# mic-rud/RABBIT-Transcoding

Hardware: AMD Instinct MI355X
Metric: transcoded point-cloud frames/sec, R5->R3 (higher is better)
Workload: dtype u16/i32

## Files before the change

rabbit-transcoding_amd/csrc/rbt_encode.h:

```cpp
#pragma once
#include "rbt_cabac.h"
#include "rbt_recon.h"
#include "rbt_filter.h"
#include "rbt_qpmap.h"

RBT_CONST uint16_t k_lambda16[76] = {3,    3,    4,    4,    5,    5,    6,    7,    8,    9,    10,   11,   12,   14,   15,   17,   19,   22,   24,
                                     27,   30,   34,   38,   43,   48,   54,   61,   68,   77,   86,   97,   108,  122,  137,  153,  172,  193,  217,
                                     244,  273,  307,  344,  387,  434,  487,  547,  614,  689,  773,  868,  974,  1093, 1227, 1378, 1546, 1736, 1948,
                                     2187, 2454, 2755, 3092, 3471, 3896, 4373, 4909, 5510, 6185, 6942, 7792, 8747, 9818, 11020, 12370, 13884, 15585, 17493};
RBT_CONST uint8_t k_intra_cand[11] = {0, 1, 26, 10, 2, 6, 14, 18, 22, 30, 34};
#define RBT_SPLIT_BITS 48
#define RBT_PARTIAL_COST 0x0FFFFFFF
#define RBT_AN_GOOD 2
#define RBT_AN_SKIPPED 0x0FFFFFFE

struct RbtEncLds {
  RbtReconLds rc;
  int16_t lvl[32 * 32];
};
struct RbtEntropyLds {
  uint8_t scan[3][4][64];
  uint8_t cu_l2[81], cu_md[81], cu_fl[81];
  alignas(16) int16_t lv[64 * 64 * 3 / 2];
};
// ... 1135 lines not shown
    while (st < 4 && (x + (st & 1) * h >= s->w || y + (st >> 1) * h >= s->h)) st++;
    if (st < 4) {
      states = (states & ~(15u << (4 * lvl))) | ((uint32_t)(st + 1) << (4 * lvl));
      x += (st & 1) * h; y += (st >> 1) * h; lg--; lvl++;
      states = (states & ~(15u << (4 * lvl))) | (15u << (4 * lvl));
    } else {
      if (lvl == 0) break;
      lvl--;
      const int k = (int)((states >> (4 * lvl)) & 15u) - 1, hh = 1 << lg;
      x -= (k & 1) * hh; y -= (k >> 1) * hh; lg++;
    }
  }
}
struct RbtSaoLds { int32_t bcnt[8][32], bsum[8][32]; int32_t ecnt[16], esum[16]; int32_t off[3][48], gain[48]; long long tgain[3][5]; int32_t bpos[3]; };
template <int TL2> struct RbtSaoRegionT { uint16_t ry[((1 << TL2) + 8) * ((1 << TL2) + 8)]; uint16_t rc[2][((1 << TL2) / 2 + 4) * ((1 << TL2) / 2 + 4)]; };
RBT_DEV int en_sao_round_div(int sum, int cnt) { return cnt ? (sum >= 0 ? sum + cnt / 2 : sum - cnt / 2) / cnt : 0; }
RBT_DEV void en_wave_sum16(const int (&v)[16], RBT_LDS_AS int32_t* dst) {
#ifdef RBT_HOSTEMU
  for (int q = 0; q < 16; q++) dst[q] = v[q];
#else
  const int lane = (int)threadIdx.x & 63, b0 = lane & 1, b1 = lane & 2;
  int a[8], b[4];
#pragma unroll
  for (int k = 0; k < 8; k++) { const int keep = b0 ? v[k + 8] : v[k], send = b0 ? v[k] : v[k + 8]; a[k] = keep + __builtin_amdgcn_update_dpp(0, send, 0xB1, 0xF, 0xF, false); }
#pragma unroll
  for (int k = 0; k < 4; k++) { const int keep = b1 ? a[k + 4] : a[k], send = b1 ? a[k] : a[k + 4]; b[k] = keep + __builtin_amdgcn_update_dpp(0, send, 0x4E, 0xF, 0xF, false); }
#pragma unroll
  for (int k = 0; k < 4; k++) {
    b[k] += __builtin_amdgcn_update_dpp(0, b[k], 0x124, 0xF, 0xF, false);
    b[k] += __builtin_amdgcn_update_dpp(0, b[k], 0x128, 0xF, 0xF, false);
    b[k] += __builtin_amdgcn_ds_swizzle(b[k], 0x401F);
    b[k] += __builtin_amdgcn_ds_bpermute((lane ^ 32) << 2, b[k]);
  }
  if (lane < 4) {
#pragma unroll
    for (int k = 0; k < 4; k++) dst[(lane & 1) * 8 + (lane & 2) * 2 + k] = b[k];
  }
#endif
}
template <bool REGION, bool QPMAP = EN_QP_ASK> RBT_DEV void en_sao_ctb(RbtFrame* f, const RbtSlice* slices, int ctb_addr, RBT_LDS_AS RbtSaoLds* L, RBT_LDS_AS uint16_t* ry, RBT_LDS_AS uint16_t* rc0, RBT_LDS_AS uint16_t* rc1) {
  const RbtStreamCfg gcopy = rc_cfg_uni(&f->cfg); const RbtStreamCfg* g = &gcopy;
  const int ctb = 1 << g->log2_ctb, cxi = ctb_addr % g->w_ctb, cyi = ctb_addr / g->w_ctb, bd = g->bit_depth, has_occ = RBT_UNI(f->occ4 != nullptr);
  const int flat = RBT_UNI(f->chroma_flat) != 0;
  EN_FLAT_COUNT(2, flat);
  const RbtSlice* sl = &slices[f->ctb_slice[ctb_addr]];
  const long long lam16 = k_lambda16[rbt_clip3(0, 75, en_ctb_qp<QPMAP>(f, sl, ctb_addr) + 6 * (bd - 8))], lam = lam16 * lam16;
  int all_skip = 0;
  if (f->ref_frame >= 0) {
    const int n8 = ctb >> 3; uint64_t m0 = 0, m1 = 0;
    RBT_VBALLOT(m0, p, rbt_min(64, n8 * n8), (cxi * n8 + p % n8 >= f->w8) || (cyi * n8 + p / n8 >= f->h8) || (f->cu_flags[(cyi * n8 + p / n8) * f->w8 + cxi * n8 + p % n8] & RBT_CU_SKIP));
    m1 = n8 * n8 >= 64 ? ~0ull : (1ull << (n8 * n8)) - 1;
    all_skip = m0 == m1;
  }
  const int lx0 = cxi * ctb, ly0 = cyi * ctb, ox = lx0 - 4, oy = ly0 - 4, cox = lx0 / 2 - 2, coy = ly0 / 2 - 2, RS = ctb + 8, RSC = ctb / 2 + 4;
  if constexpr (REGION) {
    RBT_PAR_FOR(i, RS * RS) { const int x = ox + i % RS, y = oy + i / RS; ry[i] = (x >= 0 && y >= 0 && x < g->w && y < g->h) ? f->pix[0][(size_t)y * g->w + x] : 0; }
    RBT_PAR_FOR(i, 2 * RSC * RSC) {
      const int c = i / (RSC * RSC), j = i % (RSC * RSC), x = cox + j % RSC, y = coy + j / RSC;
      (c ? rc1 : rc0)[j] = (x >= 0 && y >= 0 && x < g->cw && y < g->ch) ? f->pix[1 + c][(size_t)y * g->cw + x] : 0;
    }
    RBT_SYNC_LDS();
    for (int dir = 0; dir < 2 && REGION; dir++) {
      const int ne = ctb / 8 + 1, ns = RS / 4;
      RBT_PAR_FOR(i, ne * ns) {
        const int e = i / ns, sg = i % ns;
        const int x = dir == 0 ? lx0 + 8 * e : ox + 4 * sg, y = dir == 0 ? oy + 4 * sg : ly0 + 8 * e;
        if (x >= 0 && y >= 0 && x < g->w && y < g->h) {
          const int bs = fl_bs(f, slices, x, y, dir);
          if (bs) {
            fl_luma_core(f, slices, x, y, dir, bs, &ry[(y - oy) * RS + (x - ox)], dir == 0 ? 1 : RS, dir == 0 ? RS : 1);
            if (bs == 2 && !(dir == 0 ? (x & 15) : (y & 15)))
              for (int c = 0; c < 2; c++) fl_chroma_core(f, slices, 1 + c, x, y, dir, &(c ? rc1 : rc0)[((y >> 1) - coy) * RSC + ((x >> 1) - cox)], dir == 0 ? 1 : RSC, dir == 0 ? RSC : 1);
          }
        }
      }
      RBT_SYNC_LDS();
    }
  }
#define EN_SAO_RP(c, x, y) (REGION ? ((c) == 0 ? (int)ry[((y) - oy) * RS + ((x) - ox)] : (int)((c) == 1 ? rc0 : rc1)[((y) - coy) * RSC + ((x) - cox)]) : (int)f->pix[c][(size_t)(y) * pw + (x)])
  for (int c = 0; c < (flat ? 1 : 3) && !all_skip; c++) {
    const int sh = c ? 1 : 0, pw = c ? g->cw : g->w, ph = c ? g->ch : g->h, n = ctb >> sh, lgn = g->log2_ctb - sh;
    const int x0 = (cxi * ctb) >> sh, y0 = (cyi * ctb) >> sh;
    const uint16_t* sp = f->src[c];
    RBT_PAR_FOR(i, 8 * 32) { L->bcnt[i >> 5][i & 31] = 0; L->bsum[i >> 5][i & 31] = 0; }
    RBT_SYNC_LDS();
    int ecnt[16], esum[16];
#pragma unroll
    for (int q = 0; q < 16; q++) { ecnt[q] = 0; esum[q] = 0; }
    const int interior = !REGION && x0 > 0 && y0 > 0 && x0 + n < pw && y0 + n < ph;
    if (interior) {
#ifdef RBT_HOSTEMU
      typedef long long EnSaoAcc; const int ash = 13;
#else
      typedef int EnSaoAcc; const int ash = 7;
#endif
      EnSaoAcc acc[16];
#pragma unroll
      for (int q = 0; q < 16; q++) acc[q] = 0;
      const uint16_t* rp = f->pix[c];
      RBT_PAR_FOR(i, n * n) {
        const int x = x0 + (i & (n - 1)), y = y0 + (i >> lgn);
        if (!has_occ || en_occ_unit(f, (x << sh) >> 2, (y << sh) >> 2)) {
          const size_t o = (size_t)y * pw + x;
          const int v = rp[o], d = (int)sp[o] - v, b = rbt_min(31, v >> (bd - 5)), copy = i & 7; const EnSaoAcc dp = (EnSaoAcc)d * (1 << ash) + 1;
          RBT_LDS_ADD(&L->bcnt[copy][b], 1); RBT_LDS_ADD(&L->bsum[copy][b], d);
#pragma unroll
          for (int cls = 0; cls < 4; cls++) {
            const int step = cls == 0 ? -1 : (cls == 1 ? -pw : (cls == 2 ? -pw - 1 : -pw + 1));
            const int va = rp[o + step], vb = rp[o - step];
            const int k = 2 + (v > va) - (v < va) + (v > vb) - (v < vb), cat = k < 2 ? k : k - 1;
#pragma unroll
            for (int q = 0; q < 4; q++) acc[cls * 4 + q] += (k != 2 && cat == q) ? dp : (EnSaoAcc)0;
          }
        }
      }
#pragma unroll
      for (int q = 0; q < 16; q++) { ecnt[q] = (int)(acc[q] & ((1 << ash) - 1)); esum[q] = (int)(acc[q] >> ash); }
    } else
    RBT_PAR_FOR(i, n * n) {
      const int x = x0 + (i & (n - 1)), y = y0 + (i >> lgn);
      if (x < pw && y < ph && (!has_occ || en_occ_unit(f, (x << sh) >> 2, (y << sh) >> 2))) {
        const int v = EN_SAO_RP(c, x, y), d = (int)sp[(size_t)y * pw + x] - v, b = rbt_min(31, v >> (bd - 5)), copy = i & 7;
        RBT_LDS_ADD(&L->bcnt[copy][b], 1); RBT_LDS_ADD(&L->bsum[copy][b], d);
#pragma unroll
        for (int cls = 0; cls < 4; cls++) {
          const int dxa = cls == 1 ? 0 : (cls == 3 ? 1 : -1), dya = cls == 0 ? 0 : -1, xa = x + dxa, ya = y + dya, xb = x - dxa, yb = y - dya;
          const int inside = !(xa < 0 || ya < 0 || xb < 0 || yb < 0 || xa >= pw || xb >= pw || ya >= ph || yb >= ph);
          const int va = EN_SAO_RP(c, rbt_clip3(0, pw - 1, xa), rbt_clip3(0, ph - 1, ya)), vb = EN_SAO_RP(c, rbt_clip3(0, pw - 1, xb), rbt_clip3(0, ph - 1, yb));
          const int k = 2 + (v > va) - (v < va) + (v > vb) - (v < vb), cat = k < 2 ? k : k - 1;
#pragma unroll
          for (int q = 0; q < 4; q++) { const int hit = inside && k != 2 && cat == q; ecnt[cls * 4 + q] += hit; esum[cls * 4 + q] += hit ? d : 0; }
        }
      }
    }
    en_wave_sum16(ecnt, L->ecnt); en_wave_sum16(esum, L->esum);
    RBT_SYNC_LDS();
    RBT_PAR_FOR(j, 48) {
      int cnt, sum, o;
      if (j < 32) { cnt = 0; sum = 0; for (int q = 0; q < 8; q++) { cnt += L->bcnt[q][j]; sum += L->bsum[q][j]; } o = rbt_clip3(-7, 7, en_sao_round_div(sum, cnt)); }
      else { cnt = L->ecnt[j - 32]; sum = L->esum[j - 32]; o = en_sao_round_div(sum, cnt); o = ((j - 32) & 3) < 2 ? rbt_clip3(0, 7, o) : rbt_clip3(-7, 0, o); }
      L->off[c][j] = o; L->gain[j] = 2 * o * sum - cnt * o * o;
    }
    RBT_SYNC_LDS();
    { long long best = -1; int bp = 0;
      for (int b = 0; b <= 28; b++) { const long long gsum = (long long)L->gain[b] + L->gain[b + 1] + L->gain[b + 2] + L->gain[b + 3]; if (gsum > best) { best = gsum; bp = b; } }
      if (RBT_LANE0) { L->bpos[c] = bp; L->tgain[c][0] = best * 256 - lam * 18; } }
    for (int cls = 0; cls < 4; cls++) {
      long long gs = 0;
      for (int k = 0; k < 4; k++) gs += L->gain[32 + cls * 4 + k];
      if (RBT_LANE0) L->tgain[c][1 + cls] = gs * 256 - lam * 12;
    }
    RBT_SYNC_LDS();
  }
  RbtSao out; for (int i = 0; i < (int)sizeof(out); i++) ((uint8_t*)&out)[i] = 0;
  int bt = -1; long long bgn = 0;
  if (!all_skip) for (int t = 0; t < 5; t++) if (L->tgain[0][t] > bgn) { bgn = L->tgain[0][t]; bt = t; }
  if (bt >= 0) { out.type[0] = bt == 0 ? 1 : 2; out.band_pos[0] = (uint8_t)(bt == 0 ? L->bpos[0] : 0); out.eo_class[0] = (uint8_t)(bt ? bt - 1 : 0);
    for (int k = 0; k < 4; k++) out.offset[0][k] = (int8_t)(bt == 0 ? L->off[0][L->bpos[0] + k] : L->off[0][32 + (bt - 1) * 4 + k]); }
  bt = -1; bgn = 0;
  if (!all_skip && !flat) for (int t = 0; t < 5; t++) if (L->tgain[1][t] + L->tgain[2][t] > bgn) { bgn = L->tgain[1][t] + L->tgain[2][t]; bt = t; }
  if (bt >= 0) for (int c = 1; c < 3; c++) { out.type[c] = bt == 0 ? 1 : 2; out.band_pos[c] = (uint8_t)(bt == 0 ? L->bpos[c] : 0); out.eo_class[c] = (uint8_t)(bt ? bt - 1 : 0);
    for (int k = 0; k < 4; k++) out.offset[c][k] = (int8_t)(bt == 0 ? L->off[c][L->bpos[c] + k] : L->off[c][32 + (bt - 1) * 4 + k]); }
  { const int any0 = out.offset[0][0] | out.offset[0][1] | out.offset[0][2] | out.offset[0][3];
    const int any1 = out.offset[1][0] | out.offset[1][1] | out.offset[1][2] | out.offset[1][3], any2 = out.offset[2][0] | out.offset[2][1] | out.offset[2][2] | out.offset[2][3];
    if (!any0) out.type[0] = 0;
    if (!any1 && !any2) out.type[1] = out.type[2] = 0; }
  for (int c = 0; c < 3; c++) if (!out.type[c]) { out.band_pos[c] = 0; out.eo_class[c] = 0; for (int k = 0; k < 4; k++) out.offset[c][k] = 0; }
  if (out.type[1] != 2) out.eo_class[1] = out.eo_class[2] = 0;
  if (RBT_LANE0) f->sao[ctb_addr] = out;
  if constexpr (!REGION) rbt_sao_ctb_p(f, slices, ctb_addr, &out);
  else for (int c = 0; c < 3; c++) {
    const int sh = c ? 1 : 0, pw = c ? g->cw : g->w, ph = c ? g->ch : g->h, n = ctb >> sh, lgn = g->log2_ctb - sh, x0 = (cxi * ctb) >> sh, y0 = (cyi * ctb) >> sh;
    RBT_PAR_FOR(i, n * n) {
      const int x = x0 + (i & (n - 1)), y = y0 + (i >> lgn);
      if (x < pw && y < ph) f->out[c][(size_t)y * pw + x] = (uint16_t)rbt_sao_value(f, slices, c, x, y, &out, [&](int xx, int yy) { return EN_SAO_RP(c, xx, yy); });
    }
  }
#undef EN_SAO_RP
  RBT_SYNC_LDS();
}
struct EnSaoWords { uint64_t q[3]; };
RBT_DEV EnSaoWords en_sao_words(const RbtSao* p) {
  static_assert(sizeof(RbtSao) == 24, "three 64-bit words");
  const uint32_t* w = (const uint32_t*)p; EnSaoWords r;
  r.q[0] = (uint64_t)(uint32_t)RBT_UNI(w[0]) | ((uint64_t)(uint32_t)RBT_UNI(w[1]) << 32);
  r.q[1] = (uint64_t)(uint32_t)RBT_UNI(w[2]) | ((uint64_t)(uint32_t)RBT_UNI(w[3]) << 32);
  r.q[2] = (uint64_t)(uint32_t)RBT_UNI(w[4]) | ((uint64_t)(uint32_t)RBT_UNI(w[5]) << 32);
// ... 69 lines not shown
```

rabbit-transcoding_amd/csrc/rbt_filter.h:

```cpp
#pragma once
#include "rbt_tables.h"
#include "rbt_types.h"

RBT_DEV int fl_slice_of_ctb(const RbtFrame* f, int ctb) { const int v = f->ctb_slice[ctb]; return v == 0xFFFF ? f->first_slice : v; }
RBT_DEV int fl_slice_at(const RbtFrame* f, int x, int y) { return fl_slice_of_ctb(f, (y >> f->cfg.log2_ctb) * f->cfg.w_ctb + (x >> f->cfg.log2_ctb)); }

RBT_DEV int fl_bs(const RbtFrame* f, const RbtSlice* slices, int x, int y, int dir) {
  const RbtStreamCfg* g = &f->cfg;
  int iq = (y >> 2) * g->w4 + (x >> 2);
  int e = dir == 0 ? (f->edges[iq] & 3) : ((f->edges[iq] >> 2) & 3);
  if (!e) return 0;
  int xp = dir == 0 ? x - 1 : x, yp = dir == 0 ? y : y - 1;
  if (xp < 0 || yp < 0) return 0;
  int ip = (yp >> 2) * g->w4 + (xp >> 2);
  int sq = fl_slice_at(f, x, y), sp = fl_slice_at(f, xp, yp);
  if (slices[sq].deblocking_disabled) return 0;
  if (sp != sq && !slices[sq].lf_across) return 0;
  int mp = f->pm[ip], mq = f->pm[iq];
  if ((mp & RBT_PM_MODE_MASK) == RBT_MODE_INTRA || (mq & RBT_PM_MODE_MASK) == RBT_MODE_INTRA) return 2;
  if ((e & 1) && ((mp | mq) & RBT_PM_NZ)) return 1;
  if (f->refpoc[ip] != f->refpoc[iq]) return 1;
  if (rbt_abs(f->mv[2 * ip] - f->mv[2 * iq]) >= 4 || rbt_abs(f->mv[2 * ip + 1] - f->mv[2 * iq + 1]) >= 4) return 1;
  return 0;
}
// ... 73 lines not shown
RBT_DEV void fl_chroma_segment(RbtFrame* f, const RbtSlice* slices, int c_idx, int xl, int yl, int dir) {
  const int st = f->cfg.cw;
  fl_chroma_core(f, slices, c_idx, xl, yl, dir, f->pix[c_idx] + (size_t)(yl >> 1) * st + (xl >> 1), dir == 0 ? 1 : st, dir == 0 ? st : 1);
}
RBT_DEV int rbt_deblock_edge_count(const RbtStreamCfg* g, int dir) { return dir == 0 ? ((g->w4 + 1) >> 1) * g->h4 : g->w4 * ((g->h4 + 1) >> 1); }
RBT_DEV int rbt_deblock_edge_unit(const RbtStreamCfg* g, int dir, int e) {
  if (dir == 0) { const int hw = (g->w4 + 1) >> 1; return (e / hw) * g->w4 + 2 * (e % hw); }
  return 2 * (e / g->w4) * g->w4 + e % g->w4;
}
RBT_DEV void rbt_deblock_unit(RbtFrame* f, const RbtSlice* slices, int unit, int dir) {
  const RbtStreamCfg* g = &f->cfg;
  int x = (unit % g->w4) << 2, y = (unit / g->w4) << 2;
  if (dir == 0 ? (x & 7) : (y & 7)) return;
  int bs = fl_bs(f, slices, x, y, dir);
  if (!bs) return;
  fl_luma_segment(f, slices, x, y, dir, bs);
  if (bs == 2 && !(dir == 0 ? (x & 15) : (y & 15)) && !f->chroma_flat) { fl_chroma_segment(f, slices, 1, x, y, dir); fl_chroma_segment(f, slices, 2, x, y, dir); }
}

template <class FETCH> RBT_DEV int rbt_sao_value(const RbtFrame* f, const RbtSlice* slices, int c, int x, int y, const RbtSao* s, FETCH fetch) {
  const RbtStreamCfg* g = &f->cfg;
  int sh = c ? 1 : 0, pw = c ? g->cw : g->w, ph = c ? g->ch : g->h, bd = g->bit_depth, maxv = (1 << bd) - 1;
  int xl = x << sh, yl = y << sh;
  int ctb = (yl >> g->log2_ctb) * g->w_ctb + (xl >> g->log2_ctb);
  const RbtSlice* sl = &slices[fl_slice_of_ctb(f, ctb)];
  int v = fetch(x, y), outv = v;
  int type = s->type[c];
  if ((c ? sl->sao_chroma : sl->sao_luma) && type && !(f->pm[(yl >> 2) * g->w4 + (xl >> 2)] & RBT_PM_TQ_BYPASS)) {
    if (type == 1) {
      int band = v >> (bd - 5), k = (band - s->band_pos[c]) & 31;
      if (k < 4) outv = rbt_clip3(0, maxv, v + s->offset[c][k]);
    } else {
      int cls = s->eo_class[c];
      int dxa = cls == 1 ? 0 : (cls == 3 ? 1 : -1), dya = cls == 0 ? 0 : -1;
      int xa = x + dxa, ya = y + dya, xb = x - dxa, yb = y - dya;
      if (xa >= 0 && ya >= 0 && xb >= 0 && yb >= 0 && xa < pw && xb < pw && ya < ph && yb < ph) {
        int sa_ = fl_slice_at(f, xa << sh, ya << sh), sb_ = fl_slice_at(f, xb << sh, yb << sh), sc_ = fl_slice_of_ctb(f, ctb);
        int ok = !((sa_ != sc_ && !slices[sa_ > sc_ ? sa_ : sc_].lf_across) || (sb_ != sc_ && !slices[sb_ > sc_ ? sb_ : sc_].lf_across));
        if (ok) {
          int va = fetch(xa, ya), vb = fetch(xb, yb);
          int e = 2 + (v > va) - (v < va) + (v > vb) - (v < vb);
          if (e == 0 || e == 1 || e == 2) e = (e == 2) ? 0 : e + 1;
          if (e) outv = rbt_clip3(0, maxv, v + s->offset[c][e - 1]);
        }
      }
    }
  }
  return outv;
}
RBT_DEV void rbt_sao_sample_p(RbtFrame* f, const RbtSlice* slices, int c, int x, int y, const RbtSao* s) {
  const int pw = c ? f->cfg.cw : f->cfg.w; const uint16_t* sp = f->pix[c];
  f->out[c][(size_t)y * pw + x] = (uint16_t)rbt_sao_value(f, slices, c, x, y, s, [&](int xx, int yy) { return (int)sp[(size_t)yy * pw + xx]; });
}
RBT_DEV void rbt_sao_ctb_p(RbtFrame* f, const RbtSlice* slices, int ctb, const RbtSao* s) {
  const RbtStreamCfg* g = &f->cfg;
  const int cx = (ctb % g->w_ctb) << g->log2_ctb, cy = (ctb / g->w_ctb) << g->log2_ctb;
  const RbtSlice* sl = &slices[fl_slice_of_ctb(f, ctb)];
  const int bd = g->bit_depth, maxv = (1 << bd) - 1, bypass_possible = g->tq_bypass_enabled;
  for (int c = 0; c < 3; c++) {
    const int sh = c ? 1 : 0, pw = c ? g->cw : g->w, ph = c ? g->ch : g->h, x0 = cx >> sh, y0 = cy >> sh;
    const int nw = rbt_min((1 << g->log2_ctb) >> sh, pw - x0), nh = rbt_min((1 << g->log2_ctb) >> sh, ph - y0);
    const uint16_t* sp = f->pix[c]; uint16_t* dp = f->out[c];
    if (c && f->chroma_flat) { const uint16_t v = (uint16_t)(1 << (bd - 1)); RBT_BLK_FOR(i, nw * nh) dp[(size_t)(y0 + i / nw) * pw + x0 + i % nw] = v; continue; }
    const int type = (c ? sl->sao_chroma : sl->sao_luma) ? s->type[c] : 0;
    if (!type) { RBT_BLK_FOR(i, nw * nh) { const size_t o = (size_t)(y0 + i / nw) * pw + x0 + i % nw; dp[o] = sp[o]; } continue; }
    const int o0 = s->offset[c][0], o1 = s->offset[c][1], o2 = s->offset[c][2], o3 = s->offset[c][3];
    if (type == 1) {
      const int bp = s->band_pos[c];
      RBT_BLK_FOR(i, nw * nh) {
        const int x = x0 + i % nw, y = y0 + i / nw; const size_t o = (size_t)y * pw + x;
        const int v = sp[o], k = ((v >> (bd - 5)) - bp) & 31;
        int r = v;
        if (k < 4 && !(bypass_possible && (f->pm[((y << sh) >> 2) * g->w4 + ((x << sh) >> 2)] & RBT_PM_TQ_BYPASS))) r = rbt_clip3(0, maxv, v + (k == 0 ? o0 : (k == 1 ? o1 : (k == 2 ? o2 : o3))));
        dp[o] = (uint16_t)r;
      }
      continue;
    }
    const int cls = s->eo_class[c], dxa = cls == 1 ? 0 : (cls == 3 ? 1 : -1), dya = cls == 0 ? 0 : -1, step = dya * pw + dxa;
    const int iw = nw - 2, ih = nh - 2;
    if (iw > 0 && ih > 0) {
      RBT_BLK_FOR(i, iw * ih) {
        const int x = x0 + 1 + i % iw, y = y0 + 1 + i / iw; const size_t o = (size_t)y * pw + x;
        const int v = sp[o], va = sp[o + step], vb = sp[o - step];
        const int e = (v > va) - (v < va) + (v > vb) - (v < vb);
        int r = v;
        if (e != 0 && !(bypass_possible && (f->pm[((y << sh) >> 2) * g->w4 + ((x << sh) >> 2)] & RBT_PM_TQ_BYPASS))) r = rbt_clip3(0, maxv, v + (e == -2 ? o0 : (e == -1 ? o1 : (e == 1 ? o2 : o3))));
        dp[o] = (uint16_t)r;
      }
    }
    const int ring = iw > 0 && ih > 0 ? 2 * nw + 2 * ih : nw * nh;
    RBT_BLK_FOR(i, ring) {
      int lx, ly;
      if (!(iw > 0 && ih > 0)) { lx = i % nw; ly = i / nw; }
      else if (i < nw) { lx = i; ly = 0; }
      else if (i < 2 * nw) { lx = i - nw; ly = nh - 1; }
      else if (i < 2 * nw + ih) { lx = 0; ly = 1 + i - 2 * nw; }
      else { lx = nw - 1; ly = 1 + i - 2 * nw - ih; }
      const int x = x0 + lx, y = y0 + ly;
      dp[(size_t)y * pw + x] = (uint16_t)rbt_sao_value(f, slices, c, x, y, s, [&](int xx, int yy) { return (int)sp[(size_t)yy * pw + xx]; });
    }
  }
}
RBT_DEV void rbt_sao_ctb(RbtFrame* f, const RbtSlice* slices, int ctb) { rbt_sao_ctb_p(f, slices, ctb, &f->sao[ctb]); }
RBT_DEV void rbt_sao_sample(RbtFrame* f, const RbtSlice* slices, int c, int x, int y) {
  const RbtStreamCfg* g = &f->cfg; const int sh = c ? 1 : 0;
  rbt_sao_sample_p(f, slices, c, x, y, &f->sao[(((y << sh) >> g->log2_ctb)) * g->w_ctb + ((x << sh) >> g->log2_ctb)]);
}

#define RBT_LF_TILE 64
#define RBT_LF_R (RBT_LF_TILE + 8)
#define RBT_LF_RC (RBT_LF_TILE / 2 + 4)
struct RbtLoopLds { uint16_t y[RBT_LF_R * RBT_LF_R]; uint16_t c[2][RBT_LF_RC * RBT_LF_RC]; };
RBT_DEV void rbt_loopfilter_tile(RbtFrame* f, const RbtSlice* slices, int tile, RBT_LDS_AS RbtLoopLds* L) {
  const RbtStreamCfg* g = &f->cfg;
  const int tw = (g->w + RBT_LF_TILE - 1) / RBT_LF_TILE, x0 = (tile % tw) * RBT_LF_TILE, y0 = (tile / tw) * RBT_LF_TILE, ox = x0 - 4, oy = y0 - 4, cox = x0 / 2 - 2, coy = y0 / 2 - 2;
  RBT_BLK_FOR(i, RBT_LF_R * RBT_LF_R) { const int x = ox + i % RBT_LF_R, y = oy + i / RBT_LF_R; L->y[i] = (x >= 0 && y >= 0 && x < g->w && y < g->h) ? f->pix[0][(size_t)y * g->w + x] : 0; }
  RBT_BLK_FOR(i, 2 * RBT_LF_RC * RBT_LF_RC) {
    const int c = i / (RBT_LF_RC * RBT_LF_RC), j = i % (RBT_LF_RC * RBT_LF_RC), x = cox + j % RBT_LF_RC, y = coy + j / RBT_LF_RC;
    L->c[c][j] = (x >= 0 && y >= 0 && x < g->cw && y < g->ch) ? f->pix[1 + c][(size_t)y * g->cw + x] : 0;
  }
  RBT_SYNC();
  for (int dir = 0; dir < 2; dir++) {
    RBT_BLK_FOR(i, 9 * 18) {
      const int e = i / 18, sg = i % 18;
      const int x = dir == 0 ? x0 + 8 * e : ox + 4 * sg, y = dir == 0 ? oy + 4 * sg : y0 + 8 * e;
      if (x >= 0 && y >= 0 && x < g->w && y < g->h) {
        const int bs = fl_bs(f, slices, x, y, dir);
        if (bs) {
          fl_luma_core(f, slices, x, y, dir, bs, &L->y[(y - oy) * RBT_LF_R + (x - ox)], dir == 0 ? 1 : RBT_LF_R, dir == 0 ? RBT_LF_R : 1);
          if (bs == 2 && !(dir == 0 ? (x & 15) : (y & 15)))
            for (int c = 0; c < 2; c++) fl_chroma_core(f, slices, 1 + c, x, y, dir, &L->c[c][((y >> 1) - coy) * RBT_LF_RC + ((x >> 1) - cox)], dir == 0 ? 1 : RBT_LF_RC, dir == 0 ? RBT_LF_RC : 1);
        }
      }
    }
    RBT_SYNC();
  }
  RBT_BLK_FOR(i, RBT_LF_TILE * RBT_LF_TILE) {
    const int x = x0 + i % RBT_LF_TILE, y = y0 + i / RBT_LF_TILE;
    if (x < g->w && y < g->h) {
      const RbtSao* sp = &f->sao[(y >> g->log2_ctb) * g->w_ctb + (x >> g->log2_ctb)];
      f->out[0][(size_t)y * g->w + x] = (uint16_t)rbt_sao_value(f, slices, 0, x, y, sp, [&](int xx, int yy) { return (int)L->y[(yy - oy) * RBT_LF_R + (xx - ox)]; });
    }
  }
  RBT_BLK_FOR(i, 2 * (RBT_LF_TILE / 2) * (RBT_LF_TILE / 2)) {
    const int c = i / ((RBT_LF_TILE / 2) * (RBT_LF_TILE / 2)), j = i % ((RBT_LF_TILE / 2) * (RBT_LF_TILE / 2)), x = x0 / 2 + j % (RBT_LF_TILE / 2), y = y0 / 2 + j / (RBT_LF_TILE / 2);
    if (x < g->cw && y < g->ch) {
      const RbtSao* sp = &f->sao[((y << 1) >> g->log2_ctb) * g->w_ctb + ((x << 1) >> g->log2_ctb)];
      f->out[1 + c][(size_t)y * g->cw + x] = (uint16_t)rbt_sao_value(f, slices, 1 + c, x, y, sp, [&](int xx, int yy) { return (int)L->c[c][(yy - coy) * RBT_LF_RC + (xx - cox)]; });
    }
  }
}
```

rabbit-transcoding_amd/csrc/rbt_kernels.hip:

```cpp
#include <hip/hip_runtime.h>
#include <mutex>
#include <vector>
#include <cstdio>
#include <cstdlib>
#include "rbt_kernels.h"
#include "rbt_recon.h"
#include "rbt_filter.h"
#include "rbt_encode.h"
#include "rbt_tb_hook.h"
#include "rbt_pcc.h"

namespace rbtk {
enum { RBT_MAX_DEVICES = 16, RBT_POOL_KEEP = 160 };
struct PoolBlock { void* p; size_t n; };
struct Dev {
  int id = -1;
  hipStream_t streams[RBT_N_STREAMS] = {};
  hipEvent_t dep_ev[64]; int dep_next = 0;
  int map[RBT_N_LANES];
  hipEvent_t ev[RBT_N_LANES][16][2];
  char name[256] = "";
  std::vector<PoolBlock> pool_free, pool_live; std::mutex pool_mu;
  int depth = 1, wave_div = 2;
};
// ... 190 lines not shown
          const uint32_t* p = &q[slot - (uint32_t)n_frames]; int spins = 0;
          while ((task = __hip_atomic_load(p, __ATOMIC_RELAXED, __HIP_MEMORY_SCOPE_AGENT)) == 0) {
            __builtin_amdgcn_s_sleep(32);
            if (++spins > (1 << 20)) { refs[0].frames[refs[0].frame].error = 92; break; }
          }
        }
      }
      s_task = task;
    }
    __syncthreads();
    const uint32_t task = s_task;
    if (!task) return;
    __builtin_amdgcn_fence(__ATOMIC_ACQUIRE, "agent");
    const int fr = (int)((task - 1) >> 18), addr = (int)((task - 1) & 0x3FFFF);
    const RbtFrameRef r = refs[fr];
    RbtFrame* f = &r.frames[r.frame];
    if (f->ctb_slice[addr] != 0xFFFF) recon_ctb_roles(r.frames, r.slices, r.frame, addr, RBT_LDS_CAST(RbtReconCtbLds, &lds));
    __builtin_amdgcn_fence(__ATOMIC_RELEASE, "agent");
    asm volatile("s_waitcnt vmcnt(0)" ::: "memory");
    __syncthreads();
    if (threadIdx.x == 0) {
      const int w = f->cfg.w_ctb, h = f->cfg.h_ctb, x = addr % w, y = addr / w;
      int succ[3]; const int ns = rc_ctb_successors(w, h, x, y, succ);
      for (int k = 0; k < ns; k++) {
        const int a2 = succ[k], need = rc_ctb_need(a2 % w, a2 / w);
        if ((int)__hip_atomic_fetch_add(&f->ctb_done[2 * a2], 1u, __ATOMIC_RELAXED, __HIP_MEMORY_SCOPE_AGENT) + 1 == need) {
          const uint32_t s2 = __hip_atomic_fetch_add(tail, 1u, __ATOMIC_RELAXED, __HIP_MEMORY_SCOPE_AGENT);
          __hip_atomic_store(&q[s2], ((uint32_t)fr << 18 | (uint32_t)a2) + 1, __ATOMIC_RELAXED, __HIP_MEMORY_SCOPE_AGENT);
        }
      }
    }
  }
}
__device__ __forceinline__ int xcd_tile(int b, int n) {
  const int per = n >> 3;
  if ((gridDim.x & 7) || per == 0 || b >= per * 8) return b;
  return (b & 7) * per + (b >> 3);
}
__global__ void __launch_bounds__(256) k_deblock(RbtFrame* frames, const RbtSlice* slices, const int32_t* frame_list, int dir) {
  RbtFrame* f = &frames[frame_list[blockIdx.y]];
  const int n_edge = rbt_deblock_edge_count(&f->cfg, dir), n_blk = (n_edge + 255) >> 8;
  if ((int)blockIdx.x >= n_blk) return;
  const int e = xcd_tile(blockIdx.x, n_blk) * 256 + threadIdx.x;
  if (e >= n_edge) return;
  rbt_deblock_unit(f, slices, rbt_deblock_edge_unit(&f->cfg, dir, e), dir);
}
__global__ void __launch_bounds__(256) k_loopfilter(RbtFrame* frames, const RbtSlice* slices, const int32_t* frame_list) {
  __shared__ RbtLoopLds lds;
  RbtFrame* f = &frames[frame_list[blockIdx.y]];
  const int tw = (f->cfg.w + RBT_LF_TILE - 1) / RBT_LF_TILE, th = (f->cfg.h + RBT_LF_TILE - 1) / RBT_LF_TILE;
  if ((int)blockIdx.x >= tw * th) return;
  rbt_loopfilter_tile(f, slices, xcd_tile(blockIdx.x, tw * th), RBT_LDS_CAST(RbtLoopLds, &lds));
}
__global__ void __launch_bounds__(256) k_sao_ctb(RbtFrame* frames, const RbtSlice* slices, const int32_t* frame_list) {
  RbtFrame* f = &frames[frame_list[blockIdx.y]];
  const int n_ctb = f->cfg.w_ctb * f->cfg.h_ctb;
  if ((int)blockIdx.x >= n_ctb) return;
  rbt_sao_ctb(f, slices, xcd_tile(blockIdx.x, n_ctb));
}
__global__ void __launch_bounds__(256) k_sao(RbtFrame* frames, const RbtSlice* slices, const int32_t* frame_list) {
  RbtFrame* f = &frames[frame_list[blockIdx.y]];
  int c = blockIdx.z, pw = c ? f->cfg.cw : f->cfg.w, ph = c ? f->cfg.ch : f->cfg.h;
  const int n_blk = (pw * ph + 255) >> 8;
  if ((int)blockIdx.x >= n_blk) return;
  int i = xcd_tile(blockIdx.x, n_blk) * 256 + threadIdx.x;
  if (i >= pw * ph) return;
  rbt_sao_sample(f, slices, c, i % pw, i / pw);
}

void launch_recon(RbtFrame* frames, const RbtSlice* slices, const int32_t* frame_list, int n_frames, int max_w_ctb, int max_h_ctb, int y_begin, int y_end) {
  if (n_frames <= 0) return;
  if (y_end > max_h_ctb) y_end = max_h_ctb;
  if (y_begin >= y_end) return;
  for (int d = 2 * y_begin; d <= max_w_ctb - 1 + 2 * (y_end - 1); d++) {
    int y_hi = d / 2; if (y_hi > y_end - 1) y_hi = y_end - 1;
    int y_lo = (d - (max_w_ctb - 1) + 1) / 2; if (y_lo < y_begin) y_lo = y_begin;
    if (y_lo > y_hi) continue;
    hipLaunchKernelGGL(k_recon_diag, dim3(y_hi - y_lo + 1, n_frames), dim3(128), 0, g_stream, frames, slices, frame_list, d, y_lo);
  }
}
void launch_recon_refs(const RbtFrameRef* refs, int n_frames, int max_w_ctb, int max_h_ctb) {
  if (n_frames <= 0) return;
  for (int d = 0; d <= max_w_ctb - 1 + 2 * (max_h_ctb - 1); d++) {
    int y_hi = d / 2; if (y_hi > max_h_ctb - 1) y_hi = max_h_ctb - 1;
    int y_lo = (d - (max_w_ctb - 1) + 1) / 2; if (y_lo < 0) y_lo = 0;
    if (y_lo > y_hi) continue;
    hipLaunchKernelGGL(k_recon_diag_refs, dim3(y_hi - y_lo + 1, n_frames), dim3(128), 0, g_stream, refs, d, y_lo);
  }
}
void launch_recon_level(const RbtFrameRef* refs, int n_frames, int max_ctbs, uint32_t* ticket) {
  if (n_frames <= 0 || max_ctbs <= 0) return;
  hipLaunchKernelGGL(k_recon_level, dim3((unsigned)n_frames * (unsigned)max_ctbs), dim3(128), 0, g_stream, refs, n_frames, ticket);
}
static int g_queue_width_pct = -1;
void launch_recon_queue(const RbtFrameRef* refs, int n_frames, uint32_t total_ctbs, uint32_t* qmem, int n_wgs) {
  if (n_frames <= 0 || total_ctbs == 0) return;
  if (g_queue_width_pct < 0) { const char* e = getenv("RBT_RECON_QUEUE_WIDTH"); g_queue_width_pct = e && atoi(e) > 0 ? atoi(e) : 100; }
  long long n = (long long)n_wgs * g_queue_width_pct / 100;
  if (n < n_frames) n = n_frames; if (n > (long long)total_ctbs) n = total_ctbs; if (n > 65535 * 16) n = 65535 * 16;
  hipLaunchKernelGGL(k_recon_queue, dim3((unsigned)n), dim3(128), 0, g_stream, refs, n_frames, total_ctbs, qmem);
}
void launch_deblock(RbtFrame* frames, const RbtSlice* slices, const int32_t* frame_list, int n_frames, int max_units) {
  if (n_frames <= 0) return;
  for (int dir = 0; dir < 2; dir++)
    hipLaunchKernelGGL(k_deblock, dim3((max_units / 2 + 1024 + 255) / 256, n_frames), dim3(256), 0, g_stream, frames, slices, frame_list, dir);
}
void launch_loopfilter(RbtFrame* frames, const RbtSlice* slices, const int32_t* frame_list, int n_frames, int max_w, int max_h) {
// ... 348 lines not shown
```

rabbit-transcoding_amd/csrc/rbt_platform.h:

```cpp
#pragma once
#include <stdint.h>
#include <stddef.h>

#ifndef RBT_ABLATE
#define RBT_ABLATE 0
#endif

#ifdef RBT_HOSTEMU
#include <string.h>
#define RBT_DEV static inline
#define RBT_CONST static const
#define RBT_PAR_FOR(i, n) for (int i = 0; i < (int)(n); i++)
#define RBT_BLK_FOR(i, n) for (int i = 0; i < (int)(n); i++)
#define RBT_SYNC() do { } while (0)
#define RBT_SYNC_LDS() do { } while (0)
#define RBT_LANE0 1
#define RBT_NTHREADS 1
#define RBT_LDS_AS
#define RBT_CONST_AS
#define RBT_LDS_CAST(T, p) (p)
#define RBT_UNI(x) (x)
#define RBT_VEC(T, name) T name[64]
#define RBT_V(name, p) name[p]
#define RBT_VFOR(p, n) for (int p = 0; p < (int)(n); p++)
#define RBT_VBALLOT(out, p, n, expr) do { uint64_t b_ = 0; for (int p = 0; p < (int)(n); p++) if (expr) b_ |= 1ull << p; (out) = b_; } while (0)
#define RBT_VGET(name, lane) name[lane]
#define RBT_VSET(name, lane, v) name[lane] = (v)
#else
#include <hip/hip_runtime.h>
#define RBT_VEC(T, name) T name
#define RBT_V(name, p) name
#define RBT_VFOR(p, n) for (int p = (int)threadIdx.x & 63, once_ = 1; once_ && p < (int)(n); once_ = 0)
#define RBT_VBALLOT(out, p, n, expr) do { int p = (int)threadIdx.x & 63; (out) = __ballot(p < (int)(n) && (expr)); } while (0)
#define RBT_VGET(name, lane) __builtin_amdgcn_readlane(name, lane)
#define RBT_VSET(name, lane, v) name = rbt_writelane(name, v, lane)
__device__ int rbt_llvm_writelane(int v, int lane, int old) __asm("llvm.amdgcn.writelane");
static __device__ __forceinline__ int rbt_writelane(int old, int v, int lane) { return rbt_llvm_writelane(v, lane, old); }
#define RBT_DEV static __device__ __forceinline__
#define RBT_CONST static __device__ const
#define RBT_PAR_FOR(i, n) for (int i = (int)threadIdx.x & 63; i < (int)(n); i += 64)
#define RBT_BLK_FOR(i, n) for (int i = (int)threadIdx.x; i < (int)(n); i += (int)blockDim.x)
#define RBT_SYNC() __syncthreads()
#define RBT_SYNC_LDS() asm volatile("s_waitcnt lgkmcnt(0)" ::: "memory")
#define RBT_LANE0 ((threadIdx.x & 63) == 0)
#define RBT_NTHREADS ((int)blockDim.x)
#define RBT_LDS_AS __attribute__((address_space(3)))
#define RBT_CONST_AS __attribute__((address_space(4)))
#define RBT_LDS_CAST(T, p) ((RBT_LDS_AS T*)(uintptr_t)(p))
#ifdef RBT_NO_UNI
#define RBT_UNI(x) (x)
#else
#define RBT_UNI(x) __builtin_amdgcn_readfirstlane((int)(x))
#endif
#endif

#ifdef RBT_HOSTEMU
#define RBT_LDS_ADD(p, v) (*(p) += (v))
#else
#define RBT_LDS_ADD(p, v) ((void)__hip_atomic_fetch_add((p), (v), __ATOMIC_RELAXED, __HIP_MEMORY_SCOPE_WORKGROUP))
#endif

#ifdef RBT_HOSTEMU
#define RBT_FLAG_PUBLISH(p, v) (*(p) = (uint32_t)(v))
RBT_DEV void rbt_flag_wait(const uint32_t* p, uint32_t need, int32_t* err) { if (*p < need) *err = 91; }
RBT_DEV uint32_t rbt_flag_wait_seen(const uint32_t* p, uint32_t need, uint32_t seen, int32_t* err) { if (*p < need) *err = 91; (void)seen; return *p; }
#else
#define RBT_FLAG_PUBLISH(p, v) do { __builtin_amdgcn_fence(__ATOMIC_RELEASE, "agent"); asm volatile("s_waitcnt vmcnt(0)" ::: "memory"); \
  if (RBT_LANE0) __hip_atomic_store((p), (uint32_t)(v), __ATOMIC_RELAXED, __HIP_MEMORY_SCOPE_AGENT); } while (0)
RBT_DEV void rbt_flag_wait(const uint32_t* p, uint32_t need, int32_t* err) {
  int spins = 0;
  while (__hip_atomic_load(p, __ATOMIC_RELAXED, __HIP_MEMORY_SCOPE_AGENT) < need) {
    __builtin_amdgcn_s_sleep(32);
    if (++spins > (1 << 20)) { *err = 91; break; }
  }
  __builtin_amdgcn_fence(__ATOMIC_ACQUIRE, "agent");
}
RBT_DEV uint32_t rbt_flag_wait_seen(const uint32_t* p, uint32_t need, uint32_t seen, int32_t* err) {
  if (need <= seen) return seen;
  int spins = 0; uint32_t v;
  while ((v = __hip_atomic_load(p, __ATOMIC_RELAXED, __HIP_MEMORY_SCOPE_AGENT)) < need) {
    __builtin_amdgcn_s_sleep(32);
    if (++spins > (1 << 20)) { *err = 91; v = need; break; }
    if ((spins & 63) == 0 && __hip_atomic_load((const uint32_t*)err, __ATOMIC_RELAXED, __HIP_MEMORY_SCOPE_AGENT) != 0) { v = need; break; }
  }
  __builtin_amdgcn_fence(__ATOMIC_ACQUIRE, "agent");
  return (uint32_t)__builtin_amdgcn_readfirstlane((int)v);
}
#endif

RBT_DEV int32_t rbt_err_peek(const int32_t* err) {
#ifdef RBT_HOSTEMU
  return *err;
#else
  return __builtin_amdgcn_readfirstlane(__hip_atomic_load(err, __ATOMIC_RELAXED, __HIP_MEMORY_SCOPE_AGENT));
// ... 30 lines not shown
```

Baseline: 1033.

## Vectorize SAO apply with 4-pixel row walks and uniform scalar parameters

Rewrites the per-CTB SAO apply so each thread handles four adjacent pixels with 64-bit global loads and stores. Edge-offset classes get templated specializations, and frame and slice parameters are hoisted into scalar registers with readfirstlane. The kernel also gets a waves-per-EU occupancy hint, and host-emulation counters and cross-checks are added that compile away on the device. The aim is to cut per-pixel memory transactions and index arithmetic, at the cost of more code and a fallback path for unaligned widths.

```diff
diff --git a/rabbit-transcoding_amd/csrc/rbt_encode.h b/rabbit-transcoding_amd/csrc/rbt_encode.h
--- a/rabbit-transcoding_amd/csrc/rbt_encode.h
+++ b/rabbit-transcoding_amd/csrc/rbt_encode.h
@@ -1211,6 +1211,7 @@
     m1 = n8 * n8 >= 64 ? ~0ull : (1ull << (n8 * n8)) - 1;
     all_skip = m0 == m1;
   }
+  RBT_SAO_COUNT(32, all_skip);
   const int lx0 = cxi * ctb, ly0 = cyi * ctb, ox = lx0 - 4, oy = ly0 - 4, cox = lx0 / 2 - 2, coy = ly0 / 2 - 2, RS = ctb + 8, RSC = ctb / 2 + 4;
   if constexpr (REGION) {
     RBT_PAR_FOR(i, RS * RS) { const int x = ox + i % RS, y = oy + i / RS; ry[i] = (x >= 0 && y >= 0 && x < g->w && y < g->h) ? f->pix[0][(size_t)y * g->w + x] : 0; }
@@ -1275,7 +1276,16 @@
       }
 #pragma unroll
       for (int q = 0; q < 16; q++) { ecnt[q] = (int)(acc[q] & ((1 << ash) - 1)); esum[q] = (int)(acc[q] >> ash); }
-    } else
+    }
+    RBT_SAO_COUNT(interior ? 30 : 31, 1);
+#ifdef RBT_HOSTEMU
+    const int also_general = 1; int32_t held_b[2][8][32]; int held_e[2][16];
+    if (interior) for (int q = 0; q < 256; q++) { held_b[0][q >> 5][q & 31] = L->bcnt[q >> 5][q & 31]; held_b[1][q >> 5][q & 31] = L->bsum[q >> 5][q & 31]; L->bcnt[q >> 5][q & 31] = L->bsum[q >> 5][q & 31] = 0; }
+    if (interior) for (int q = 0; q < 16; q++) { held_e[0][q] = ecnt[q]; held_e[1][q] = esum[q]; ecnt[q] = esum[q] = 0; }
+#else
+    const int also_general = 0;
+#endif
+    if (!interior || also_general)
     RBT_PAR_FOR(i, n * n) {
       const int x = x0 + (i & (n - 1)), y = y0 + (i >> lgn);
       if (x < pw && y < ph && (!has_occ || en_occ_unit(f, (x << sh) >> 2, (y << sh) >> 2))) {
@@ -1292,6 +1302,14 @@
         }
       }
     }
+#ifdef RBT_HOSTEMU
+    if (interior) {
+      int differ = 0;
+      for (int q = 0; q < 256; q++) differ |= held_b[0][q >> 5][q & 31] != L->bcnt[q >> 5][q & 31] || held_b[1][q >> 5][q & 31] != L->bsum[q >> 5][q & 31];
+      for (int q = 0; q < 16; q++) differ |= held_e[0][q] != ecnt[q] || held_e[1][q] != esum[q];
+      RBT_SAO_COUNT(33, 1); RBT_SAO_COUNT(34, differ);
+    }
+#endif
     en_wave_sum16(ecnt, L->ecnt); en_wave_sum16(esum, L->esum);
     RBT_SYNC_LDS();
     RBT_PAR_FOR(j, 48) {
diff --git a/rabbit-transcoding_amd/csrc/rbt_filter.h b/rabbit-transcoding_amd/csrc/rbt_filter.h
--- a/rabbit-transcoding_amd/csrc/rbt_filter.h
+++ b/rabbit-transcoding_amd/csrc/rbt_filter.h
@@ -149,43 +149,118 @@
   const int pw = c ? f->cfg.cw : f->cfg.w; const uint16_t* sp = f->pix[c];
   f->out[c][(size_t)y * pw + x] = (uint16_t)rbt_sao_value(f, slices, c, x, y, s, [&](int xx, int yy) { return (int)sp[(size_t)yy * pw + xx]; });
 }
+#ifdef RBT_HOSTEMU
+extern "C" { inline uint32_t rbt_hostemu_sao_walk[35]; }
+#define RBT_SAO_COUNT(k, n) ((void)__atomic_fetch_add(&rbt_hostemu_sao_walk[k], (uint32_t)(n), __ATOMIC_RELAXED))
+#else
+#define RBT_SAO_COUNT(k, n) do { } while (0)
+#endif
+struct RbtPx4 { uint32_t lo, hi; };
+RBT_DEV RbtPx4 rbt_px4_load(const RBT_GLOBAL_AS uint16_t* p) {
+#ifdef RBT_HOSTEMU
+  RbtPx4 r; memcpy(&r, p, 8); return r;
+#else
+  typedef uint32_t rbt_u32x2 __attribute__((ext_vector_type(2)));
+  const rbt_u32x2 t = *(const RBT_GLOBAL_AS rbt_u32x2*)p; RbtPx4 r; r.lo = t.x; r.hi = t.y; return r;
+#endif
+}
+RBT_DEV void rbt_px4_store(RBT_GLOBAL_AS uint16_t* p, RbtPx4 v) {
+#ifdef RBT_HOSTEMU
+  memcpy(p, &v, 8);
+#else
+  typedef uint32_t rbt_u32x2 __attribute__((ext_vector_type(2)));
+  rbt_u32x2 t; t.x = v.lo; t.y = v.hi; *(RBT_GLOBAL_AS rbt_u32x2*)p = t;
+#endif
+}
+RBT_DEV void rbt_px4_unpack(RbtPx4 p, int (&v)[4]) { v[0] = (int)(p.lo & 0xFFFFu); v[1] = (int)(p.lo >> 16); v[2] = (int)(p.hi & 0xFFFFu); v[3] = (int)(p.hi >> 16); }
+RBT_DEV RbtPx4 rbt_px4_pack(const int (&v)[4]) { RbtPx4 p; p.lo = (uint32_t)v[0] | ((uint32_t)v[1] << 16); p.hi = (uint32_t)v[2] | ((uint32_t)v[3] << 16); return p; }
+struct RbtSaoWalk {
+  const RBT_GLOBAL_AS uint16_t* sp; RBT_GLOBAL_AS uint16_t* dp; const uint8_t* pm;
+  int pw, x0, y0, nw, nh, lgw, sh, w4, bd, maxv, bypass_possible, o0, o1, o2, o3;
+};
+RBT_DEV uint32_t rbt_sao_walk_at(const RbtSaoWalk& k, int lx, int ly) { return (uint32_t)(k.y0 + ly) * (uint32_t)k.pw + (uint32_t)(k.x0 + lx); }
+RBT_DEV int rbt_sao_walk_bypass(const RbtSaoWalk& k, int lx, int ly) { return k.pm[(((k.y0 + ly) << k.sh) >> 2) * k.w4 + (((k.x0 + lx) << k.sh) >> 2)] & RBT_PM_TQ_BYPASS; }
+template <int DXA, int DYA> RBT_DEV void rbt_sao_walk_edge(const RbtSaoWalk& k) {
+  static_assert(DYA == 0 || DYA == -1, "a is the neighbour in the row above, or in the same row");
+  RBT_ROW_WALK(gi, yy, k.lgw, k.nh - 2) {
+    const int lx = gi << 2, ly = 1 + yy;
+    if (lx >= k.nw) continue;
+    const uint32_t oc = rbt_sao_walk_at(k, lx, ly), oa = DYA ? oc - (uint32_t)k.pw : oc, ob = DYA ? oc + (uint32_t)k.pw : oc;
+    int v[4], a[4], b[4];
+    const RbtPx4 pc = rbt_px4_load(k.sp + oc);
+    rbt_px4_unpack(pc, v);
+    if constexpr (DXA == 0) { rbt_px4_unpack(rbt_px4_load(k.sp + oa), a); rbt_px4_unpack(rbt_px4_load(k.sp + ob), b); }
+    else {
+      int ra[4], rb[4];
+      rbt_px4_unpack(DYA ? rbt_px4_load(k.sp + oa) : pc, ra); rbt_px4_unpack(DYA ? rbt_px4_load(k.sp + ob) : pc, rb);
+      const uint32_t left = (uint32_t)(lx > 0), right = lx + 4 < k.nw ? 4u : 3u;
+      if constexpr (DXA < 0) { const int ea = k.sp[oa - left], eb = k.sp[ob + right]; a[0] = ea; a[1] = ra[0]; a[2] = ra[1]; a[3] = ra[2]; b[0] = rb[1]; b[1] = rb[2]; b[2] = rb[3]; b[3] = eb; }
+      else { const int ea = k.sp[oa + right], eb = k.sp[ob - left]; a[0] = ra[1]; a[1] = ra[2]; a[2] = ra[3]; a[3] = ea; b[0] = eb; b[1] = rb[0]; b[2] = rb[1]; b[3] = rb[2]; }
+    }
+    int r[4];
+#pragma unroll
+    for (int j = 0; j < 4; j++) {
+      const int e = (v[j] > a[j]) - (v[j] < a[j]) + (v[j] > b[j]) - (v[j] < b[j]);
+      r[j] = v[j];
+      if (e != 0 && !(k.bypass_possible && rbt_sao_walk_bypass(k, lx + j, ly))) r[j] = rbt_clip3(0, k.maxv, v[j] + (e == -2 ? k.o0 : (e == -1 ? k.o1 : (e == 1 ? k.o2 : k.o3))));
+    }
+    if (lx > 0 && lx + 4 < k.nw) rbt_px4_store(k.dp + oc, rbt_px4_pack(r));
+    else {
+#pragma unroll
+      for (int j = 0; j < 4; j++) if (lx + j >= 1 && lx + j <= k.nw - 2) k.dp[oc + (uint32_t)j] = (uint16_t)r[j];
+    }
+  }
+}
 RBT_DEV void rbt_sao_ctb_p(RbtFrame* f, const RbtSlice* slices, int ctb, const RbtSao* s) {
   const RbtStreamCfg* g = &f->cfg;
-  const int cx = (ctb % g->w_ctb) << g->log2_ctb, cy = (ctb / g->w_ctb) << g->log2_ctb;
-  const RbtSlice* sl = &slices[fl_slice_of_ctb(f, ctb)];
-  const int bd = g->bit_depth, maxv = (1 << bd) - 1, bypass_possible = g->tq_bypass_enabled;
+  const int log2_ctb = RBT_UNI(g->log2_ctb), w_ctb = RBT_UNI(g->w_ctb), bd = RBT_UNI(g->bit_depth);
+  const int cx = (ctb % w_ctb) << log2_ctb, cy = (ctb / w_ctb) << log2_ctb;
+  const RbtSlice* sl = &slices[RBT_UNI(fl_slice_of_ctb(f, ctb))];
+  const int sao_luma = RBT_UNI(sl->sao_luma), sao_chroma = RBT_UNI(sl->sao_chroma), flat = RBT_UNI(f->chroma_flat) != 0;
+  RbtSaoWalk k;
+  k.pm = rbt_uni_ptr(f->pm); k.w4 = RBT_UNI(g->w4); k.bd = bd; k.maxv = (1 << bd) - 1; k.bypass_possible = RBT_UNI(g->tq_bypass_enabled); k.o0 = k.o1 = k.o2 = k.o3 = 0;
   for (int c = 0; c < 3; c++) {
-    const int sh = c ? 1 : 0, pw = c ? g->cw : g->w, ph = c ? g->ch : g->h, x0 = cx >> sh, y0 = cy >> sh;
-    const int nw = rbt_min((1 << g->log2_ctb) >> sh, pw - x0), nh = rbt_min((1 << g->log2_ctb) >> sh, ph - y0);
-    const uint16_t* sp = f->pix[c]; uint16_t* dp = f->out[c];
-    if (c && f->chroma_flat) { const uint16_t v = (uint16_t)(1 << (bd - 1)); RBT_BLK_FOR(i, nw * nh) dp[(size_t)(y0 + i / nw) * pw + x0 + i % nw] = v; continue; }
-    const int type = (c ? sl->sao_chroma : sl->sao_luma) ? s->type[c] : 0;
-    if (!type) { RBT_BLK_FOR(i, nw * nh) { const size_t o = (size_t)(y0 + i / nw) * pw + x0 + i % nw; dp[o] = sp[o]; } continue; }
-    const int o0 = s->offset[c][0], o1 = s->offset[c][1], o2 = s->offset[c][2], o3 = s->offset[c][3];
+    const int sh = c ? 1 : 0, pw = RBT_UNI(c ? g->cw : g->w), ph = RBT_UNI(c ? g->ch : g->h), x0 = cx >> sh, y0 = cy >> sh, n = (1 << log2_ctb) >> sh;
+    const int nw = rbt_min(n, pw - x0), nh = rbt_min(n, ph - y0);
+    k.sp = (const RBT_GLOBAL_AS uint16_t*)rbt_uni_ptr(f->pix[c]); k.dp = (RBT_GLOBAL_AS uint16_t*)rbt_uni_ptr(f->out[c]);
+    k.pw = pw; k.x0 = x0; k.y0 = y0; k.nw = nw; k.nh = nh; k.sh = sh; k.lgw = log2_ctb - sh - 2;
+    const int type = (c ? sao_chroma : sao_luma) ? RBT_UNI(s->type[c]) : 0, cls = RBT_UNI(s->eo_class[c]);
+    const int fill = c && flat; const uint16_t fv = (uint16_t)(1 << (bd - 1));
+    RBT_SAO_COUNT(10 * c + 8, nw < n); RBT_SAO_COUNT(10 * c + 9, nh < n);
+    RBT_SAO_COUNT(10 * c + (fill ? 6 : (type == 0 ? 0 : (type == 1 ? 1 : 2 + cls))), 1);
+    auto fetch = [&](int xx, int yy) { return (int)k.sp[(uint32_t)yy * (uint32_t)pw + (uint32_t)xx]; };
+    if ((pw | x0 | nw) & 3) {
+      RBT_BLK_FOR(i, nw * nh) { const int lx = i % nw, ly = i / nw; k.dp[rbt_sao_walk_at(k, lx, ly)] = fill ? fv : (uint16_t)rbt_sao_value(f, slices, c, x0 + lx, y0 + ly, s, fetch); }
+      continue;
+    }
+    if (fill) { RbtPx4 v4; v4.lo = v4.hi = (uint32_t)fv * 0x10001u; RBT_ROW_WALK(gi, ly, k.lgw, nh) { if ((gi << 2) < nw) rbt_px4_store(k.dp + rbt_sao_walk_at(k, gi << 2, ly), v4); } continue; }
+    if (!type) { RBT_ROW_WALK(gi, ly, k.lgw, nh) { if ((gi << 2) < nw) { const uint32_t o = rbt_sao_walk_at(k, gi << 2, ly); rbt_px4_store(k.dp + o, rbt_px4_load(k.sp + o)); } } continue; }
+    k.o0 = RBT_UNI(s->offset[c][0]); k.o1 = RBT_UNI(s->offset[c][1]); k.o2 = RBT_UNI(s->offset[c][2]); k.o3 = RBT_UNI(s->offset[c][3]);
     if (type == 1) {
-      const int bp = s->band_pos[c];
-      RBT_BLK_FOR(i, nw * nh) {
-        const int x = x0 + i % nw, y = y0 + i / nw; const size_t o = (size_t)y * pw + x;
-        const int v = sp[o], k = ((v >> (bd - 5)) - bp) & 31;
-        int r = v;
-        if (k < 4 && !(bypass_possible && (f->pm[((y << sh) >> 2) * g->w4 + ((x << sh) >> 2)] & RBT_PM_TQ_BYPASS))) r = rbt_clip3(0, maxv, v + (k == 0 ? o0 : (k == 1 ? o1 : (k == 2 ? o2 : o3))));
-        dp[o] = (uint16_t)r;
+      const int bp = RBT_UNI(s->band_pos[c]);
+      RBT_ROW_WALK(gi, ly, k.lgw, nh) {
+        const int lx = gi << 2;
+        if (lx >= nw) continue;
+        const uint32_t o = rbt_sao_walk_at(k, lx, ly);
+        int v[4]; rbt_px4_unpack(rbt_px4_load(k.sp + o), v);
+#pragma unroll
+        for (int j = 0; j < 4; j++) {
+          const int q = ((v[j] >> (bd - 5)) - bp) & 31;
+          if (q < 4 && !(k.bypass_possible && rbt_sao_walk_bypass(k, lx + j, ly))) v[j] = rbt_clip3(0, k.maxv, v[j] + (q == 0 ? k.o0 : (q == 1 ? k.o1 : (q == 2 ? k.o2 : k.o3))));
+        }
+        rbt_px4_store(k.dp + o, rbt_px4_pack(v));
       }
       continue;
     }
-    const int cls = s->eo_class[c], dxa = cls == 1 ? 0 : (cls == 3 ? 1 : -1), dya = cls == 0 ? 0 : -1, step = dya * pw + dxa;
     const int iw = nw - 2, ih = nh - 2;
     if (iw > 0 && ih > 0) {
-      RBT_BLK_FOR(i, iw * ih) {
-        const int x = x0 + 1 + i % iw, y = y0 + 1 + i / iw; const size_t o = (size_t)y * pw + x;
-        const int v = sp[o], va = sp[o + step], vb = sp[o - step];
-        const int e = (v > va) - (v < va) + (v > vb) - (v < vb);
-        int r = v;
-        if (e != 0 && !(bypass_possible && (f->pm[((y << sh) >> 2) * g->w4 + ((x << sh) >> 2)] & RBT_PM_TQ_BYPASS))) r = rbt_clip3(0, maxv, v + (e == -2 ? o0 : (e == -1 ? o1 : (e == 1 ? o2 : o3))));
-        dp[o] = (uint16_t)r;
-      }
+      if (cls == 0) rbt_sao_walk_edge<-1, 0>(k);
+      else if (cls == 1) rbt_sao_walk_edge<0, -1>(k);
+      else if (cls == 2) rbt_sao_walk_edge<-1, -1>(k);
+      else rbt_sao_walk_edge<1, -1>(k);
     }
     const int ring = iw > 0 && ih > 0 ? 2 * nw + 2 * ih : nw * nh;
+    RBT_SAO_COUNT(10 * c + 7, ring);
     RBT_BLK_FOR(i, ring) {
       int lx, ly;
       if (!(iw > 0 && ih > 0)) { lx = i % nw; ly = i / nw; }
@@ -193,8 +268,7 @@
       else if (i < 2 * nw) { lx = i - nw; ly = nh - 1; }
       else if (i < 2 * nw + ih) { lx = 0; ly = 1 + i - 2 * nw; }
       else { lx = nw - 1; ly = 1 + i - 2 * nw - ih; }
-      const int x = x0 + lx, y = y0 + ly;
-      dp[(size_t)y * pw + x] = (uint16_t)rbt_sao_value(f, slices, c, x, y, s, [&](int xx, int yy) { return (int)sp[(size_t)yy * pw + xx]; });
+      k.dp[rbt_sao_walk_at(k, lx, ly)] = (uint16_t)rbt_sao_value(f, slices, c, x0 + lx, y0 + ly, s, fetch);
     }
   }
 }
diff --git a/rabbit-transcoding_amd/csrc/rbt_kernels.hip b/rabbit-transcoding_amd/csrc/rbt_kernels.hip
--- a/rabbit-transcoding_amd/csrc/rbt_kernels.hip
+++ b/rabbit-transcoding_amd/csrc/rbt_kernels.hip
@@ -266,7 +266,7 @@
   if ((int)blockIdx.x >= tw * th) return;
   rbt_loopfilter_tile(f, slices, xcd_tile(blockIdx.x, tw * th), RBT_LDS_CAST(RbtLoopLds, &lds));
 }
-__global__ void __launch_bounds__(256) k_sao_ctb(RbtFrame* frames, const RbtSlice* slices, const int32_t* frame_list) {
+__global__ void __launch_bounds__(256) __attribute__((amdgpu_waves_per_eu(8))) k_sao_ctb(RbtFrame* frames, const RbtSlice* slices, const int32_t* frame_list) {
   RbtFrame* f = &frames[frame_list[blockIdx.y]];
   const int n_ctb = f->cfg.w_ctb * f->cfg.h_ctb;
   if ((int)blockIdx.x >= n_ctb) return;
diff --git a/rabbit-transcoding_amd/csrc/rbt_platform.h b/rabbit-transcoding_amd/csrc/rbt_platform.h
--- a/rabbit-transcoding_amd/csrc/rbt_platform.h
+++ b/rabbit-transcoding_amd/csrc/rbt_platform.h
@@ -12,6 +12,8 @@
 #define RBT_CONST static const
 #define RBT_PAR_FOR(i, n) for (int i = 0; i < (int)(n); i++)
 #define RBT_BLK_FOR(i, n) for (int i = 0; i < (int)(n); i++)
+#define RBT_ROW_WALK(g, y, lgw, nh) for (int i_ = 0, g = 0, y = 0; y < (int)(nh); i_++, g = i_ & ((1 << (lgw)) - 1), y = i_ >> (lgw))
+#define RBT_GLOBAL_AS
 #define RBT_SYNC() do { } while (0)
 #define RBT_SYNC_LDS() do { } while (0)
 #define RBT_LANE0 1
@@ -40,6 +42,8 @@
 #define RBT_CONST static __device__ const
 #define RBT_PAR_FOR(i, n) for (int i = (int)threadIdx.x & 63; i < (int)(n); i += 64)
 #define RBT_BLK_FOR(i, n) for (int i = (int)threadIdx.x; i < (int)(n); i += (int)blockDim.x)
+#define RBT_ROW_WALK(g, y, lgw, nh) for (int g = (int)threadIdx.x & ((1 << (lgw)) - 1), y = (int)threadIdx.x >> (lgw); y < (int)(nh); y += (int)blockDim.x >> (lgw))
+#define RBT_GLOBAL_AS __attribute__((address_space(1)))
 #define RBT_SYNC() __syncthreads()
 #define RBT_SYNC_LDS() asm volatile("s_waitcnt lgkmcnt(0)" ::: "memory")
 #define RBT_LANE0 ((threadIdx.x & 63) == 0)
```

Result: no change. 1042, median of 5 (+0.9%).
